# autonomousvision/unimatch

Measured on NVIDIA B200. Metric: image-pairs/sec @480x832 gmflow-scale2-refine6; EPE vs reference, higher is better.
Workload: dtype fp32

## Files before the change

include/unimatch_sm100.h:

```cpp
#ifndef UNIMATCH_SM100_H_
#define UNIMATCH_SM100_H_

#include <stdint.h>

#ifdef __cplusplus
extern "C" {
#endif

#define UM_OK 0
#define UM_EINVAL (-22)
#define UM_ECUDA (-5)

#define UM_FEATURE_DIM 128

int um_abi_version(void);
const char* um_build_info(void);
const char* um_last_error(void);
int64_t um_launch_count(void);

#define UM_MASK_NONE 0
#define UM_MASK_SWIN 1
#define UM_MASK_CAUSAL 2

typedef struct um_attn_geom {
// ... 7 lines not shown
                        int32_t n_streams, int32_t kv_shift,
                        int64_t ldq, int64_t ldk, int64_t ldv, int64_t ldo,
                        const um_attn_geom* geom, void* workspace, int64_t workspace_bytes, int32_t flags,
                        void* stream);
#define UM_ATTN_FORCE_CUDA_CORES 1
int64_t um_window_attention_workspace(const um_attn_geom* geom, int32_t n_streams);
void um_debug_set_dump(float* device_buffer);

int32_t um_attention_planes_lp(const um_attn_geom* geom);
int um_window_attention_planes(const void* q_planes, const void* k_planes, const void* v_planes, float* out, int64_t ldo,
                               void* out_split, int64_t split_plane_stride, int32_t n_streams, int32_t kv_shift,
                               const um_attn_geom* geom, void* stream);

#define UM_VALUE_TENSOR 0
#define UM_VALUE_COORDS 1
#define UM_VALUE_XCOORD 2
#define UM_POST_NONE 0
#define UM_POST_MINUS_OWN 1
#define UM_POST_OWN_MINUS 2

int um_softmax_expectation(const float* q, const float* k, const float* values, float* out,
                           int32_t n_streams, int32_t n_total, int32_t kv_shift,
                           int64_t ldq, int64_t ldk, int32_t vdim, int32_t value_mode, int32_t post_op,
                           const um_attn_geom* geom, void* workspace, int64_t workspace_bytes, int32_t flags,
                           void* stream);
int64_t um_softmax_expectation_workspace(const um_attn_geom* geom, int32_t n_total, int32_t value_mode);

int um_local_corr_softmax(const float* f0, const float* f1, float* flow,
                          int32_t batch, int32_t h, int32_t w, int32_t ry, int32_t rx, int32_t stereo,
                          void* stream);

int um_local_corr_volume(const float* f0, const float* f1, const float* flow, float* corr,
                         int32_t batch, int32_t h, int32_t w, int32_t radius, int32_t flow_dim, void* stream);

int um_flow_warp(const float* f, const float* flow, float* out,
                 int32_t batch, int32_t h, int32_t w, int32_t flow_dim, void* stream);

int um_fb_consistency(const float* fwd_flow, const float* bwd_flow, float alpha, float beta, float* fwd_occ,
                      float* bwd_occ, int32_t batch, int32_t h, int32_t w, void* stream);

int um_propagate_local(const float* q, const float* k, const float* flow, float* out,
                       int32_t batch, int32_t h, int32_t w, int32_t radius, int32_t flow_dim,
                       int64_t ldq, int64_t ldk, void* stream);

int um_depth_corr_softmax(const float* f0, const float* f1, const float* Kmat, const float* Kinv,
                          const float* pose, const float* cand, float* out,
                          int32_t batch, int32_t h, int32_t w, int32_t num_cand, int32_t from_argmax,
                          void* stream);

int um_add_position(const float* x, const float* table, float* out,
                    int32_t n_streams, int32_t h, int32_t w, int32_t wh, int32_t ww, void* stream);

int um_layernorm_residual(const float* x, const float* residual, const float* gamma, const float* beta,
                          float* out, int64_t rows, int64_t ldx, int64_t ldr, int64_t ldo, void* stream);

int um_convex_upsample(const float* flow, const float* mask, float* up,
                       int32_t batch, int32_t h, int32_t w, int32_t flow_dim, int32_t factor, float mult,
                       void* stream);

int um_upsample2x(const float* flow, float* out, int32_t batch, int32_t h, int32_t w, int32_t flow_dim,
                  float mult, void* stream);

int um_resize_bilinear(const float* in, float* out, int32_t batch, int32_t channels, int32_t h_in, int32_t w_in,
                       int32_t h_out, int32_t w_out, const float* scale, int32_t flip_x, void* stream);

int um_gru_rh(const float* r_pre, int64_t ldr, const float* h, int64_t ldh, float* rh, int64_t ldo, int64_t rows,
// ... 83 lines not shown
```

unimatch_b200/csrc/build.py:

```python
import hashlib
import os
import shutil
import subprocess
import sys

HERE = os.path.dirname(os.path.abspath(__file__))
ROOT = os.path.dirname(os.path.dirname(HERE))
LIB = os.path.join(os.path.dirname(HERE), "libunimatch_sm100.so")
SOURCES = ["um_api.cu", "um_attention_simt.cu", "um_attention_tc.cu", "um_attention_tc2.cu", "um_conv_tc.cu", "um_ffn_tc.cu", "um_local.cu", "um_local_stencil.cu", "um_misc.cu", "um_norm.cu", "um_stem.cu"]
FLAGS = ["-gencode", "arch=compute_100a,code=sm_100a", "-O3", "-lineinfo", "-std=c++17",
         "-Xcompiler", "-fPIC", "-Xcompiler", "-O2", "-I", os.path.join(ROOT, "include"), "-I", HERE]


def _nvcc():
    for c in (shutil.which("nvcc"), "/usr/local/cuda/bin/nvcc"):
        if c and os.path.exists(c):
            return c
    raise RuntimeError("nvcc not found: libunimatch_sm100.so cannot be built")


def have_nvcc():
    try:
        _nvcc()
        return True
    except RuntimeError:
        return False


if os.environ.get("UM_ATTN_DEBUG_BUILD") == "1":
    FLAGS = FLAGS + ["-DUM_ATTN_DEBUG=1"]


def _stamp():
    h = hashlib.sha256()
    h.update(" ".join(FLAGS).replace(ROOT, "").encode())
    for f in sorted(os.listdir(HERE)) + [os.path.join(ROOT, "include", "unimatch_sm100.h")]:
        p = f if os.path.isabs(f) else os.path.join(HERE, f)
        if p.endswith((".cu", ".cuh", ".h", "build.py")):
            h.update(open(p, "rb").read())
    return h.hexdigest()


# ... 55 lines not shown
```

unimatch_b200/csrc/um_local.cu:

```cuda
#include <limits.h>
#include <math_constants.h>

#include "um_common.cuh"

namespace {

constexpr float SQRT_C = 11.313708498984761f;
constexpr int PIX_PER_CTA = 32;

struct Tap { int x0, y0; float wnw, wne, wsw, wse; };

__device__ __forceinline__ float unnormalize(float g, int size) { return ((g + 1.0f) / 2.0f) * (float)(size - 1); }

__device__ __forceinline__ float norm_sample(float p, int size) { return 2.0f * p / (float)(size - 1) - 1.0f; }
__device__ __forceinline__ float norm_window(float p, int size) { float c = (float)(size - 1) / 2.0f; return (p - c) / c; }

__device__ __forceinline__ Tap make_tap(float ix, float iy) {
  Tap t;
  float fx = floorf(ix), fy = floorf(iy);
  t.x0 = (int)fx; t.y0 = (int)fy;
  float xe = fx + 1.0f, ye = fy + 1.0f;
  t.wnw = (xe - ix) * (ye - iy);
  t.wne = (ix - fx) * (ye - iy);
  t.wsw = (xe - ix) * (iy - fy);
  t.wse = (ix - fx) * (iy - fy);
  return t;
}

struct Vec16 { float4 v[4]; };

__device__ __forceinline__ Vec16 load_row(const float* row, int sub) {
  Vec16 r;
  const float4* p = reinterpret_cast<const float4*>(row);
#pragma unroll
  for (int i = 0; i < 4; ++i) r.v[i] = __ldg(p + sub + 8 * i);
  return r;
}
__device__ __forceinline__ void store_row(float* row, int sub, const Vec16& r) {
  float4* p = reinterpret_cast<float4*>(row);
#pragma unroll
  for (int i = 0; i < 4; ++i) p[sub + 8 * i] = r.v[i];
}
__device__ __forceinline__ Vec16 zero16() {
  Vec16 r;
#pragma unroll
  for (int i = 0; i < 4; ++i) r.v[i] = make_float4(0.f, 0.f, 0.f, 0.f);
  return r;
}
__device__ __forceinline__ void axpy(Vec16& acc, float w, const Vec16& x) {
#pragma unroll
  for (int i = 0; i < 4; ++i) {
    acc.v[i].x = fmaf(w, x.v[i].x, acc.v[i].x); acc.v[i].y = fmaf(w, x.v[i].y, acc.v[i].y);
    acc.v[i].z = fmaf(w, x.v[i].z, acc.v[i].z); acc.v[i].w = fmaf(w, x.v[i].w, acc.v[i].w);
  }
}
__device__ __forceinline__ float dot_partial(const Vec16& a, const Vec16& b) {
  float s = 0.f;
#pragma unroll
  for (int i = 0; i < 4; ++i) {
    s = fmaf(a.v[i].x, b.v[i].x, s); s = fmaf(a.v[i].y, b.v[i].y, s);
    s = fmaf(a.v[i].z, b.v[i].z, s); s = fmaf(a.v[i].w, b.v[i].w, s);
  }
  return s;
}
__device__ __forceinline__ float reduce8(float s) {
  const unsigned gmask = 0xFFu << (threadIdx.x & 24);
  s += __shfl_xor_sync(gmask, s, 4);
  s += __shfl_xor_sync(gmask, s, 2);
  s += __shfl_xor_sync(gmask, s, 1);
  return s;
}

__device__ __forceinline__ Vec16 sample(const float* img, int h, int w, const Tap& t, int sub) {
  Vec16 acc = zero16();
  const bool xl = (t.x0 >= 0 && t.x0 < w), xr = (t.x0 + 1 >= 0 && t.x0 + 1 < w);
  const bool yt = (t.y0 >= 0 && t.y0 < h), yb = (t.y0 + 1 >= 0 && t.y0 + 1 < h);
  if (yt && xl && t.wnw != 0.0f) axpy(acc, t.wnw, load_row(img + ((long long)t.y0 * w + t.x0) * UM_C, sub));
  if (yt && xr && t.wne != 0.0f) axpy(acc, t.wne, load_row(img + ((long long)t.y0 * w + t.x0 + 1) * UM_C, sub));
  if (yb && xl && t.wsw != 0.0f) axpy(acc, t.wsw, load_row(img + ((long long)(t.y0 + 1) * w + t.x0) * UM_C, sub));
  if (yb && xr && t.wse != 0.0f) axpy(acc, t.wse, load_row(img + ((long long)(t.y0 + 1) * w + t.x0 + 1) * UM_C, sub));
  return acc;
}

__device__ __forceinline__ void read_flow(const float* flow, long long pix, int flow_dim, float* u, float* v) {
  if (flow_dim == 2) { float2 f = __ldg(reinterpret_cast<const float2*>(flow) + pix); *u = f.x; *v = f.y; }
  else { *u = -__ldg(flow + pix); *v = 0.0f; }
}

__global__ void __launch_bounds__(256) flow_warp_kernel(const float* __restrict__ f, const float* __restrict__ flow,
                                                        float* __restrict__ out, int h, int w, int flow_dim,
                                                        long long npix) {
  const int sub = threadIdx.x & 7;
  const long long pix = (long long)blockIdx.x * PIX_PER_CTA + (threadIdx.x >> 3);
  if (pix >= npix) return;
  const long long hw = (long long)h * w;
  const int b = (int)(pix / hw);
  const int rem = (int)(pix - (long long)b * hw);
  const int y = rem / w, x = rem - y * w;
  float u, v;
  read_flow(flow, pix, flow_dim, &u, &v);
  const float px = (float)x + u, py = (float)y + v;
  Tap t = make_tap(unnormalize(norm_sample(px, w), w), unnormalize(norm_sample(py, h), h));
  Vec16 r = sample(f + (long long)b * hw * UM_C, h, w, t, sub);
  store_row(out + pix * UM_C, sub, r);
}

__global__ void __launch_bounds__(256) local_corr_softmax_kernel(const float* __restrict__ f0, const float* __restrict__ f1,
                                                                 float* __restrict__ out, int h, int w, int ry, int rx,
                                                                 int stereo, long long npix) {
  const int sub = threadIdx.x & 7;
  const long long pix = (long long)blockIdx.x * PIX_PER_CTA + (threadIdx.x >> 3);
  if (pix >= npix) return;
  const long long hw = (long long)h * w;
  const int b = (int)(pix / hw);
  const int rem = (int)(pix - (long long)b * hw);
  const int y = rem / w, x = rem - y * w;
  const Vec16 a = load_row(f0 + pix * UM_C, sub);
  const float* img = f1 + (long long)b * hw * UM_C;
  float m = -CUDART_INF_F, l = 0.f, ax = 0.f, ay = 0.f;
// ... 275 lines not shown
```

unimatch_b200/ops.py:

```python
import ctypes
import os

import torch

_HERE = os.path.dirname(os.path.abspath(__file__))
LIB_PATH = os.path.join(_HERE, "libunimatch_sm100.so")

SYMBOLS = [
    "um_abi_version", "um_build_info", "um_last_error", "um_launch_count",
    "um_window_attention", "um_window_attention_workspace", "um_attention_planes_lp", "um_window_attention_planes", "um_debug_set_dump", "um_softmax_expectation", "um_softmax_expectation_workspace",
    "um_local_corr_softmax", "um_local_corr_volume", "um_flow_warp", "um_fb_consistency", "um_propagate_local", "um_depth_corr_softmax",
    "um_conv2d_tc", "um_ffn_tc", "um_conv7x7_small", "um_split_planes", "um_instance_norm_scratch_floats", "um_instance_norm_stats", "um_instance_norm_apply", "um_add_position", "um_layernorm_residual", "um_convex_upsample", "um_upsample2x", "um_resize_bilinear", "um_gru_rh", "um_gru_update",
]

MASK_NONE, MASK_SWIN, MASK_CAUSAL = 0, 1, 2
VALUE_TENSOR, VALUE_COORDS, VALUE_XCOORD = 0, 1, 2
POST_NONE, POST_MINUS_OWN, POST_OWN_MINUS = 0, 1, 2


FORCE_CUDA_CORES = 1
_force_cuda_cores = False


def set_force_cuda_cores(flag):
    global _force_cuda_cores
    _force_cuda_cores = bool(flag)


ACT_NONE, ACT_RELU, ACT_TANH, ACT_SIGMOID, ACT_GELU = 0, 1, 2, 3, 4
CONV_LINEAR, CONV_GRU_ZR, CONV_GRU_Q, CONV_LN = 0, 1, 2, 3


class AttnGeom(ctypes.Structure):
    _fields_ = [(n, ctypes.c_int32) for n in ("h", "w", "kh", "kw", "sh", "sw", "mask_mode")]


class ConvDesc(ctypes.Structure):
    _fields_ = [("src", ctypes.c_void_p * 2), ("cin_p", ctypes.c_int32 * 2), ("nsrc", ctypes.c_int32),
                ("batch", ctypes.c_int32), ("h", ctypes.c_int32), ("w", ctypes.c_int32),
                ("weights", ctypes.c_void_p), ("bias", ctypes.c_void_p),
                ("kh", ctypes.c_int32), ("kw", ctypes.c_int32), ("pad_h", ctypes.c_int32), ("pad_w", ctypes.c_int32),
                ("cout", ctypes.c_int32), ("cout_p", ctypes.c_int32), ("bn", ctypes.c_int32),
                ("mode", ctypes.c_int32), ("act", ctypes.c_int32),
                ("out_f32", ctypes.c_void_p), ("ld_f32", ctypes.c_int64), ("off_f32", ctypes.c_int32),
# ... 5 lines not shown
                ("win_dst", ctypes.c_void_p), ("win_c0", ctypes.c_int32), ("win_c1", ctypes.c_int32),
                ("win_lp", ctypes.c_int32), ("win_streams", ctypes.c_int32), ("win_geom", AttnGeom),
                ("pre", ctypes.c_void_p), ("ld_pre", ctypes.c_int64)]


class FfnDesc(ctypes.Structure):
    _fields_ = [("src", ctypes.c_void_p * 2), ("src_plane_stride", ctypes.c_int64), ("rows", ctypes.c_int64),
                ("w1", ctypes.c_void_p), ("w2", ctypes.c_void_p), ("hidden", ctypes.c_int32),
                ("residual", ctypes.c_void_p), ("ld_res", ctypes.c_int64), ("gamma", ctypes.c_void_p), ("beta", ctypes.c_void_p),
                ("out_f32", ctypes.c_void_p), ("ld_f32", ctypes.c_int64), ("out_split", ctypes.c_void_p),
                ("split_plane_stride", ctypes.c_int64)]


def _load():
    from .csrc.build import build, have_nvcc
    if have_nvcc():
        build()
    elif not os.path.exists(LIB_PATH):
        raise ImportError("libunimatch_sm100.so is missing and nvcc is not available to build it")
    lib = ctypes.CDLL(LIB_PATH)
    missing = [s for s in SYMBOLS if not hasattr(lib, s)]
    if missing:
        raise ImportError("libunimatch_sm100.so lacks symbols %s (stale build? run python unimatch_b200/csrc/build.py --force)" % missing)
    lib.um_build_info.restype = ctypes.c_char_p
    lib.um_last_error.restype = ctypes.c_char_p
    lib.um_launch_count.restype = ctypes.c_int64
    P, I, L, F = ctypes.c_void_p, ctypes.c_int32, ctypes.c_int64, ctypes.c_float
    G = ctypes.POINTER(AttnGeom)
    sig = {
        "um_window_attention": [P, P, P, P, I, I, L, L, L, L, G, P, L, I, P],
        "um_softmax_expectation": [P, P, P, P, I, I, I, L, L, I, I, I, G, P, L, I, P],
        "um_local_corr_softmax": [P, P, P, I, I, I, I, I, I, P],
        "um_local_corr_volume": [P, P, P, P, I, I, I, I, I, P],
        "um_flow_warp": [P, P, P, I, I, I, I, P],
        "um_fb_consistency": [P, P, F, F, P, P, I, I, I, P],
        "um_propagate_local": [P, P, P, P, I, I, I, I, I, L, L, P],
        "um_depth_corr_softmax": [P, P, P, P, P, P, P, I, I, I, I, I, P],
        "um_add_position": [P, P, P, I, I, I, I, I, P],
        "um_layernorm_residual": [P, P, P, P, P, L, L, L, L, P],
        "um_convex_upsample": [P, P, P, I, I, I, I, I, F, P],
        "um_upsample2x": [P, P, I, I, I, I, F, P],
        "um_gru_rh": [P, L, P, L, P, L, L, P],
        "um_gru_update": [P, L, P, L, P, L, P, L, L, P],
    }
    lib.um_window_attention_workspace.argtypes = [G, I]
    lib.um_window_attention_workspace.restype = ctypes.c_int64
    lib.um_softmax_expectation_workspace.argtypes = [G, I, I]
    lib.um_softmax_expectation_workspace.restype = ctypes.c_int64
    lib.um_conv2d_tc.argtypes = [ctypes.POINTER(ConvDesc), P]
    lib.um_conv2d_tc.restype = ctypes.c_int
    lib.um_ffn_tc.argtypes = [ctypes.POINTER(FfnDesc), P]
    lib.um_ffn_tc.restype = ctypes.c_int
    lib.um_split_planes.argtypes = [P, L, I, L, P, I, I, L, P]
    lib.um_attention_planes_lp.argtypes = [G]
    lib.um_attention_planes_lp.restype = ctypes.c_int32
    lib.um_window_attention_planes.argtypes = [P, P, P, P, L, P, L, I, I, G, P]
    lib.um_window_attention_planes.restype = ctypes.c_int
    lib.um_split_planes.restype = ctypes.c_int
    FP = ctypes.POINTER(ctypes.c_float)
    lib.um_conv7x7_small.argtypes = [P, P, I, I, I, I, I, I, I, P, P, I, I, FP, FP, P, L, P, I, P]
    lib.um_conv7x7_small.restype = ctypes.c_int
    lib.um_instance_norm_scratch_floats.argtypes = [I, I]
    lib.um_instance_norm_scratch_floats.restype = ctypes.c_int64
    lib.um_instance_norm_stats.argtypes = [P, L, I, I, I, P, P, P]
    lib.um_instance_norm_stats.restype = ctypes.c_int
    lib.um_instance_norm_apply.argtypes = [P, L, P, I, P, L, P, I, P, L, P, I, I, I, I, I, P]
# ... 134 lines not shown
    return out


softmax_expectation = _define(
    "softmax_expectation(Tensor q, Tensor k, Tensor? values, int n_streams, int kv_shift, int vdim, int value_mode, "
    "int post_op, int h, int w, int kh, int kw, int mask_mode) -> Tensor", _softmax_expectation)


def _local_corr_softmax(f0, f1, h, w, ry, rx, stereo):
    _f32c(f0, "f0"), _f32c(f1, "f1")
    b = f0.shape[0]
    out = torch.empty((b, h, w, 1 if stereo else 2), device=f0.device, dtype=torch.float32)
    _check(LIB.um_local_corr_softmax(_p(f0), _p(f1), _p(out), b, h, w, ry, rx, int(stereo), _stream()),
           "um_local_corr_softmax")
    return out


local_corr_softmax = _define("local_corr_softmax(Tensor f0, Tensor f1, int h, int w, int ry, int rx, bool stereo) -> Tensor",
                             _local_corr_softmax)


def _local_corr_volume(f0, f1, flow, h, w, radius):
    _f32c(f0, "f0"), _f32c(f1, "f1"), _f32c(flow, "flow")
    b = f0.shape[0]
    k = (2 * radius + 1) ** 2
    out = torch.empty((b, h, w, k), device=f0.device, dtype=torch.float32)
    _check(LIB.um_local_corr_volume(_p(f0), _p(f1), _p(flow), _p(out), b, h, w, radius, flow.shape[-1], _stream()),
           "um_local_corr_volume")
    return out


local_corr_volume = _define("local_corr_volume(Tensor f0, Tensor f1, Tensor flow, int h, int w, int radius) -> Tensor",
                            _local_corr_volume)


def _flow_warp(f, flow, h, w):
    _f32c(f, "f"), _f32c(flow, "flow")
    out = torch.empty_like(f)
    _check(LIB.um_flow_warp(_p(f), _p(flow), _p(out), f.shape[0], h, w, flow.shape[-1], _stream()), "um_flow_warp")
    return out


flow_warp = _define("flow_warp(Tensor f, Tensor flow, int h, int w) -> Tensor", _flow_warp)


def _fb_consistency(fwd_flow, bwd_flow, alpha, beta):
    _f32c(fwd_flow, "fwd_flow"), _f32c(bwd_flow, "bwd_flow")
    if fwd_flow.dim() != 4 or fwd_flow.shape[1] != 2 or fwd_flow.shape != bwd_flow.shape:
        raise ValueError("fb_consistency: flows must be planar [B,2,H,W] of equal shape")
    b, _, h, w = fwd_flow.shape
    fwd_occ = torch.empty((b, h, w), device=fwd_flow.device, dtype=torch.float32)
    bwd_occ = torch.empty_like(fwd_occ)
    _check(LIB.um_fb_consistency(_p(fwd_flow), _p(bwd_flow), float(alpha), float(beta), _p(fwd_occ), _p(bwd_occ), b, h, w,
                                 _stream()), "um_fb_consistency")
    return fwd_occ, bwd_occ


fb_consistency = _define("fb_consistency(Tensor fwd_flow, Tensor bwd_flow, float alpha, float beta) -> (Tensor, Tensor)",
                         _fb_consistency)


def _propagate_local(q, k, flow, h, w, radius):
    ldq, ldk = _rows(q, "q"), _rows(k, "k")
    _f32c(flow, "flow")
    b = q.shape[0]
    out = torch.empty_like(flow)
# ... 299 lines not shown
```

unimatch_b200/unimatch.py:

```python
import math
from contextlib import contextmanager

import torch
import torch.nn as nn

from . import ops
from .spec import param_spec

_OPS = torch.ops.unimatch_sm100


import os as _os
_FUSED_FFN = _os.environ.get("UM_FUSED_FFN", "1") != "0"


def _bn256(b, h, w):
    return 128 if (b * ((h + 7) // 8) * ((w + 15) // 16)) % 2 == 0 else 256



class _Node(nn.Module):
    """Parameter container; gives the flat spec table the reference's dotted state_dict names."""


def _attach(root, key, param):
    parts = key.split(".")
    node = root
    for name in parts[:-1]:
        if name not in node._modules:
            node.add_module(name, _Node())
        node = node._modules[name]
    node.register_parameter(parts[-1], param)


def _sine_table(wh, ww):
    y = torch.arange(1, wh + 1, dtype=torch.float32)
    x = torch.arange(1, ww + 1, dtype=torch.float32)
    y = y / (float(wh) + 1e-6) * (2 * math.pi)
    x = x / (float(ww) + 1e-6) * (2 * math.pi)
    n = torch.arange(64, dtype=torch.float32)
    dim_t = 10000 ** (2 * torch.div(n, 2, rounding_mode="floor") / 64)
    even = (torch.arange(64) % 2 == 0)

    def enc(v):
        a = v[:, None] / dim_t
        return torch.where(even, a.sin(), a.cos())
# ... 398 lines not shown
                                        ops.VALUE_TENSOR, ops.POST_NONE, h, wd, 1, 1, ops.MASK_NONE).view(nb, h, wd, fd)

    class _RefineState:
        pass

    def _stage_refine_setup(self, P, feat0, b, h, w):
        T = P["tc"]
        dev = feat0.device
        st = self._RefineState()
        z16 = lambda cp: torch.empty((2, b, h, w, cp), device=dev, dtype=torch.float16)
        st.corr_s = self._zero_padded("corr", (2, b, h, w, 128), dev)
        st.cor1_s, st.cf_s, st.flo1_s = z16(256), z16(256), z16(128)
        st.inp_s, st.mfx_s = z16(128), z16(128)
        st.h0_s, st.h1_s, st.h2_s, st.rh_s, st.fh_s = z16(128), z16(128), z16(128), z16(128), z16(256)
        f0_s = z16(128)
        _OPS.split_planes(feat0, f0_s, 0)
        f32 = lambda cc: torch.empty((b, h, w, cc), device=dev)
        st.net0, st.z, st.h1, st.h2 = f32(128), f32(128), f32(128), f32(128)
        C, LIN, NONE = self._conv, ops.CONV_LINEAR, ops.ACT_NONE
        C(f0_s, None, *T["proj_net"], 1, 1, 0, 0, 128, 128, LIN, ops.ACT_TANH, st.net0, 0, st.h0_s, 0, None, None)
        C(f0_s, None, *T["proj_inp"], 1, 1, 0, 0, 128, 128, LIN, ops.ACT_RELU, None, 0, st.inp_s, 0, None, None)
        st.pre_zr1, st.pre_q1, st.pre_zr2, st.pre_q2 = f32(256), f32(128), f32(256), f32(128)
        bn_zr = _bn256(b, h, w)
        C(st.h0_s, st.inp_s, *T["zr1_fix"], 1, 5, 0, 2, 256, bn_zr, LIN, NONE, st.pre_zr1, 0, None, 0, None, None)
        C(st.inp_s, None, *T["q1_fix"], 1, 5, 0, 2, 128, 128, LIN, NONE, st.pre_q1, 0, None, 0, None, None)
        C(st.inp_s, None, *T["zr2_fix"], 5, 1, 2, 0, 256, bn_zr, LIN, NONE, st.pre_zr2, 0, None, 0, None, None)
        C(st.inp_s, None, *T["q2_fix"], 5, 1, 2, 0, 128, 128, LIN, NONE, st.pre_q2, 0, None, 0, None, None)
        return st

    def _update_block(self, P, st, corr, flow, want_mask):
        T, w = P["tc"], P["raw"]
        fd = T["fd"]
        C, L, R = self._conv, ops.CONV_LINEAR, ops.ACT_RELU
        b, h, wd, _ = corr.shape
        dev = corr.device
        bn_zr = bn_fh = _bn256(b, h, wd)
        _OPS.split_planes(corr, st.corr_s, 0)
        C(st.corr_s, None, *T["convc1"], 1, 1, 0, 0, 256, 256, L, R, None, 0, st.cor1_s, 0, None, None)
        C(st.cor1_s, None, *T["convc2"], 3, 3, 1, 1, 192, 96 if bn_zr == 128 else 192, L, R, None, 0, st.cf_s, 0, None, None)
        _OPS.conv7x7_small(flow, None, False, w["refine.encoder.convf1.weight"], w["refine.encoder.convf1.bias"], 1, True,
                           None, None, None, st.flo1_s)
        C(st.flo1_s, None, *T["convf2"], 3, 3, 1, 1, 64, 64, L, R, None, 0, st.cf_s, 192, None, None)
        C(st.cf_s, None, *T["conv"], 3, 3, 1, 1, 128 - fd, 128, L, R, None, 0, st.mfx_s, 0, None, None)
        _OPS.split_planes(flow, st.mfx_s, 128 - fd)
        Z, Q = ops.CONV_GRU_ZR, ops.CONV_GRU_Q
        kw = dict(gamma=None, beta=None, stride=1, rows=0, win_dst=None, win_geom=None, win_c0=0, win_c1=0, win_streams=0)
        C(st.mfx_s, None, T["zr1_var"], None, 1, 5, 0, 2, 256, bn_zr, Z, 0, st.z, 0, st.rh_s, 0, st.net0, None, pre=st.pre_zr1, **kw)
        C(st.rh_s, st.mfx_s, T["q1_var"], None, 1, 5, 0, 2, 128, 128, Q, 0, st.h1, 0, st.h1_s, 0, st.net0, st.z, pre=st.pre_q1, **kw)
        C(st.h1_s, st.mfx_s, T["zr2_var"], None, 5, 1, 2, 0, 256, bn_zr, Z, 0, st.z, 0, st.rh_s, 0, st.h1, None, pre=st.pre_zr2, **kw)
        C(st.rh_s, st.mfx_s, T["q2_var"], None, 5, 1, 2, 0, 128, 128, Q, 0, st.h2, 0, st.h2_s, 0, st.h1, st.z, pre=st.pre_q2, **kw)
        C(st.h2_s, None, *T["fh1"], 3, 3, 1, 1, 256, bn_fh, L, R, None, 0, st.fh_s, 0, None, None)
        delta = torch.empty((b, h, wd, fd), device=dev)
        C(st.fh_s, None, *T["fh2"], 3, 3, 1, 1, fd, 16, L, ops.ACT_NONE, delta, 0, None, 0, None, None)
        mask = None
        if want_mask and "mask0" in T:
            C(st.h2_s, None, *T["mask0"], 3, 3, 1, 1, 256, bn_fh, L, R, None, 0, st.fh_s, 0, None, None)
            nm = w["refine.mask.2.weight"].shape[0]
            mask = torch.empty((b, h, wd, nm), device=dev)
            C(st.fh_s, None, *T["mask2"], 1, 1, 0, 0, nm, 64, L, ops.ACT_NONE, mask, 0, None, 0, None, None)
        return st.h2, mask, delta

    def _stage_refine_iter(self, P, rst, g0, g1, flow, task, want_mask, depth=None):
        h, wd = flow.shape[1], flow.shape[2]
        if task == "depth":
            Kr, pr, min_depth, max_depth = depth
            cflow = self._rigid_flow(flow, Kr.float(), pr.float(), h, wd)
        else:
            cflow = flow.contiguous()
        with self._section("refine_corr_volume"):
            corr = _OPS.local_corr_volume(g0, g1, cflow, h, wd, 4)
        with self._section("refine_update_block"):
            _, mask, delta = self._update_block(P, rst, corr, flow.contiguous(), want_mask)
        if task == "depth":
            flow = (flow - delta).clamp(min=min_depth, max=max_depth)
        else:
            flow = flow + delta
        if task == "stereo":
            flow = flow.clamp(min=0)
        return flow, mask

    def _stage_upsample_learned(self, P, flow2, feat, factor, mult):
        U = P["up"]
        b, h, w, _ = feat.shape
        dev = feat.device
        C = self._conv
        src = self._zero_padded("upsampler", (2, b, h, w, 192), dev)
        _OPS.split_planes(feat.contiguous(), src, 0)
        _OPS.split_planes(flow2.contiguous(), src, 128)
        mid = torch.empty((2, b, h, w, 256), device=dev, dtype=torch.float16)
        C(src, None, *U["c0"], 3, 3, 1, 1, 256, _bn256(b, h, w), ops.CONV_LINEAR, ops.ACT_RELU, None, 0, mid, 0, None, None)
        m = torch.empty((b, h, w, U["nm"]), device=dev)
        C(mid, None, *U["c2"], 1, 1, 0, 0, U["nm"], U["bn2"], ops.CONV_LINEAR, ops.ACT_NONE, m, 0, None, 0, None, None)
        return _OPS.convex_upsample(flow2.contiguous(), m, factor, float(mult))

    @staticmethod
    def _rigid_flow(inv_depth, K, pose, h, w):
        b = inv_depth.shape[0]
        dev = inv_depth.device
        ys, xs = torch.meshgrid(torch.arange(h, device=dev, dtype=torch.float32),
                                torch.arange(w, device=dev, dtype=torch.float32), indexing="ij")
        grid = torch.stack([xs, ys, torch.ones_like(xs)], dim=0).view(1, 3, -1).expand(b, 3, h * w)
        depth = (1.0 / inv_depth.view(b, 1, h * w))
        pts = torch.inverse(K).bmm(grid) * depth
# ... 114 lines not shown
```

Measured before the change: 157.1.

## Compute refine local correlation volume on tensor cores from fp16 split planes

```diff
diff --git a/include/unimatch_sm100.h b/include/unimatch_sm100.h
--- a/include/unimatch_sm100.h
+++ b/include/unimatch_sm100.h
@@ -63,6 +63,9 @@
 
 int um_local_corr_volume(const float* f0, const float* f1, const float* flow, float* corr,
                          int32_t batch, int32_t h, int32_t w, int32_t radius, int32_t flow_dim, void* stream);
+int um_local_corr_volume_planes(const void* f0_planes, const void* f1_planes, const float* flow, float* corr,
+                                void* out_split, int32_t cp_split, int32_t off_split, int32_t batch, int32_t h, int32_t w,
+                                int32_t radius, int32_t flow_dim, int32_t* fallback_tiles, void* stream);
 
 int um_flow_warp(const float* f, const float* flow, float* out,
                  int32_t batch, int32_t h, int32_t w, int32_t flow_dim, void* stream);
diff --git a/unimatch_b200/csrc/build.py b/unimatch_b200/csrc/build.py
--- a/unimatch_b200/csrc/build.py
+++ b/unimatch_b200/csrc/build.py
@@ -7,7 +7,7 @@
 HERE = os.path.dirname(os.path.abspath(__file__))
 ROOT = os.path.dirname(os.path.dirname(HERE))
 LIB = os.path.join(os.path.dirname(HERE), "libunimatch_sm100.so")
-SOURCES = ["um_api.cu", "um_attention_simt.cu", "um_attention_tc.cu", "um_attention_tc2.cu", "um_conv_tc.cu", "um_ffn_tc.cu", "um_local.cu", "um_local_stencil.cu", "um_misc.cu", "um_norm.cu", "um_stem.cu"]
+SOURCES = ["um_api.cu", "um_attention_simt.cu", "um_attention_tc.cu", "um_attention_tc2.cu", "um_conv_tc.cu", "um_ffn_tc.cu", "um_local.cu", "um_local_tc.cu", "um_local_stencil.cu", "um_misc.cu", "um_norm.cu", "um_stem.cu"]
 FLAGS = ["-gencode", "arch=compute_100a,code=sm_100a", "-O3", "-lineinfo", "-std=c++17",
          "-Xcompiler", "-fPIC", "-Xcompiler", "-O2", "-I", os.path.join(ROOT, "include"), "-I", HERE]
 
diff --git a/unimatch_b200/csrc/um_local.cu b/unimatch_b200/csrc/um_local.cu
--- a/unimatch_b200/csrc/um_local.cu
+++ b/unimatch_b200/csrc/um_local.cu
@@ -2,40 +2,14 @@
 #include <math_constants.h>
 
 #include "um_common.cuh"
+#include "um_local_tap.cuh"
 
 namespace {
 
-constexpr float SQRT_C = 11.313708498984761f;
+using namespace um::local;
+
 constexpr int PIX_PER_CTA = 32;
 
-struct Tap { int x0, y0; float wnw, wne, wsw, wse; };
-
-__device__ __forceinline__ float unnormalize(float g, int size) { return ((g + 1.0f) / 2.0f) * (float)(size - 1); }
-
-__device__ __forceinline__ float norm_sample(float p, int size) { return 2.0f * p / (float)(size - 1) - 1.0f; }
-__device__ __forceinline__ float norm_window(float p, int size) { float c = (float)(size - 1) / 2.0f; return (p - c) / c; }
-
-__device__ __forceinline__ Tap make_tap(float ix, float iy) {
-  Tap t;
-  float fx = floorf(ix), fy = floorf(iy);
-  t.x0 = (int)fx; t.y0 = (int)fy;
-  float xe = fx + 1.0f, ye = fy + 1.0f;
-  t.wnw = (xe - ix) * (ye - iy);
-  t.wne = (ix - fx) * (ye - iy);
-  t.wsw = (xe - ix) * (iy - fy);
-  t.wse = (ix - fx) * (iy - fy);
-  return t;
-}
-
-struct Vec16 { float4 v[4]; };
-
-__device__ __forceinline__ Vec16 load_row(const float* row, int sub) {
-  Vec16 r;
-  const float4* p = reinterpret_cast<const float4*>(row);
-#pragma unroll
-  for (int i = 0; i < 4; ++i) r.v[i] = __ldg(p + sub + 8 * i);
-  return r;
-}
 __device__ __forceinline__ void store_row(float* row, int sub, const Vec16& r) {
   float4* p = reinterpret_cast<float4*>(row);
 #pragma unroll
@@ -54,23 +28,6 @@
     acc.v[i].z = fmaf(w, x.v[i].z, acc.v[i].z); acc.v[i].w = fmaf(w, x.v[i].w, acc.v[i].w);
   }
 }
-__device__ __forceinline__ float dot_partial(const Vec16& a, const Vec16& b) {
-  float s = 0.f;
-#pragma unroll
-  for (int i = 0; i < 4; ++i) {
-    s = fmaf(a.v[i].x, b.v[i].x, s); s = fmaf(a.v[i].y, b.v[i].y, s);
-    s = fmaf(a.v[i].z, b.v[i].z, s); s = fmaf(a.v[i].w, b.v[i].w, s);
-  }
-  return s;
-}
-__device__ __forceinline__ float reduce8(float s) {
-  const unsigned gmask = 0xFFu << (threadIdx.x & 24);
-  s += __shfl_xor_sync(gmask, s, 4);
-  s += __shfl_xor_sync(gmask, s, 2);
-  s += __shfl_xor_sync(gmask, s, 1);
-  return s;
-}
-
 __device__ __forceinline__ Vec16 sample(const float* img, int h, int w, const Tap& t, int sub) {
   Vec16 acc = zero16();
   const bool xl = (t.x0 >= 0 && t.x0 < w), xr = (t.x0 + 1 >= 0 && t.x0 + 1 < w);
@@ -80,11 +37,6 @@
   if (yb && xl && t.wsw != 0.0f) axpy(acc, t.wsw, load_row(img + ((long long)(t.y0 + 1) * w + t.x0) * UM_C, sub));
   if (yb && xr && t.wse != 0.0f) axpy(acc, t.wse, load_row(img + ((long long)(t.y0 + 1) * w + t.x0 + 1) * UM_C, sub));
   return acc;
-}
-
-__device__ __forceinline__ void read_flow(const float* flow, long long pix, int flow_dim, float* u, float* v) {
-  if (flow_dim == 2) { float2 f = __ldg(reinterpret_cast<const float2*>(flow) + pix); *u = f.x; *v = f.y; }
-  else { *u = -__ldg(flow + pix); *v = 0.0f; }
 }
 
 __global__ void __launch_bounds__(256) flow_warp_kernel(const float* __restrict__ f, const float* __restrict__ flow,
diff --git a/unimatch_b200/csrc/um_local_tap.cuh b/unimatch_b200/csrc/um_local_tap.cuh
--- /dev/null
+++ b/unimatch_b200/csrc/um_local_tap.cuh
@@ -0,0 +1,76 @@
+#pragma once
+#include "um_common.cuh"
+
+namespace um {
+namespace local {
+
+constexpr float SQRT_C = 11.313708498984761f;
+
+struct Tap { int x0, y0; float wnw, wne, wsw, wse; };
+
+__device__ __forceinline__ float unnormalize(float g, int size) { return ((g + 1.0f) / 2.0f) * (float)(size - 1); }
+
+__device__ __forceinline__ float norm_sample(float p, int size) { return 2.0f * p / (float)(size - 1) - 1.0f; }
+__device__ __forceinline__ float norm_window(float p, int size) { float c = (float)(size - 1) / 2.0f; return (p - c) / c; }
+
+__device__ __forceinline__ Tap make_tap(float ix, float iy) {
+  Tap t;
+  float fx = floorf(ix), fy = floorf(iy);
+  t.x0 = (int)fx; t.y0 = (int)fy;
+  float xe = fx + 1.0f, ye = fy + 1.0f;
+  t.wnw = (xe - ix) * (ye - iy);
+  t.wne = (ix - fx) * (ye - iy);
+  t.wsw = (xe - ix) * (iy - fy);
+  t.wse = (ix - fx) * (iy - fy);
+  return t;
+}
+
+__device__ __forceinline__ void read_flow(const float* flow, long long pix, int flow_dim, float* u, float* v) {
+  if (flow_dim == 2) { float2 f = __ldg(reinterpret_cast<const float2*>(flow) + pix); *u = f.x; *v = f.y; }
+  else { *u = -__ldg(flow + pix); *v = 0.0f; }
+}
+
+__device__ __forceinline__ Tap corr_center_tap(const float* flow, long long pix, int flow_dim, int x, int y, int h, int w) {
+  float u, v;
+  read_flow(flow, pix, flow_dim, &u, &v);
+  const float cx = unnormalize(norm_window((float)x + u, w), w);
+  const float cy = unnormalize(norm_window((float)y + v, h), h);
+  return make_tap(cx, cy);
+}
+
+__device__ __forceinline__ float blend(float nw, float ne, float sw, float se, const Tap& t) {
+  float r = nw * t.wnw;
+  r = fmaf(ne, t.wne, r);
+  r = fmaf(sw, t.wsw, r);
+  r = fmaf(se, t.wse, r);
+  return r / SQRT_C;
+}
+
+struct Vec16 { float4 v[4]; };
+
+__device__ __forceinline__ Vec16 load_row(const float* row, int sub) {
+  Vec16 r;
+  const float4* p = reinterpret_cast<const float4*>(row);
+#pragma unroll
+  for (int i = 0; i < 4; ++i) r.v[i] = __ldg(p + sub + 8 * i);
+  return r;
+}
+__device__ __forceinline__ float dot_partial(const Vec16& a, const Vec16& b) {
+  float s = 0.f;
+#pragma unroll
+  for (int i = 0; i < 4; ++i) {
+    s = fmaf(a.v[i].x, b.v[i].x, s); s = fmaf(a.v[i].y, b.v[i].y, s);
+    s = fmaf(a.v[i].z, b.v[i].z, s); s = fmaf(a.v[i].w, b.v[i].w, s);
+  }
+  return s;
+}
+__device__ __forceinline__ float reduce8(float s) {
+  const unsigned gmask = 0xFFu << (threadIdx.x & 24);
+  s += __shfl_xor_sync(gmask, s, 4);
+  s += __shfl_xor_sync(gmask, s, 2);
+  s += __shfl_xor_sync(gmask, s, 1);
+  return s;
+}
+
+}
+}
diff --git a/unimatch_b200/csrc/um_local_tc.cu b/unimatch_b200/csrc/um_local_tc.cu
--- /dev/null
+++ b/unimatch_b200/csrc/um_local_tc.cu
@@ -0,0 +1,387 @@
+#include <limits.h>
+
+#include "um_common.cuh"
+#include "um_local_tap.cuh"
+#include "um_tc.cuh"
+
+namespace um {
+
+using namespace tc;
+using namespace local;
+
+namespace {
+
+constexpr int TW = 16, TH = 8;
+constexpr int R = 4, GRID = 2 * R + 2, NOUT = (2 * R + 1) * (2 * R + 1);
+constexpr int CW = 32, CH = 8;
+constexpr int CSTEP = CW - GRID + 1;
+constexpr int MAX_CHUNKS = 6;
+constexpr int MAX_SPREAD = 256;
+constexpr int STAGES = 2;
+constexpr int NEPI = 8;
+constexpr int NTHREADS = 64 + 32 * NEPI;
+constexpr int INFO_SLOTS = 4;
+constexpr int ROWBUF_LD = 33;
+constexpr uint32_t A_BYTES = 4 * 16384;
+constexpr uint32_t STAGE_BYTES = 32768;
+constexpr uint32_t STAGING_BYTES = 128 * NOUT * 4;
+constexpr uint32_t ROWBUF_BYTES = NEPI * 32 * ROWBUF_LD * 4;
+constexpr uint32_t TAIL_BYTES = 256;
+constexpr uint32_t SMEM_BYTES = A_BYTES + STAGES * STAGE_BYTES + STAGING_BYTES + ROWBUF_BYTES + TAIL_BYTES;
+static_assert(SMEM_BYTES <= 232448, "shared memory budget");
+
+struct TileInfo { int X0, Y0, nr, nc; };
+
+struct CorrParams {
+  int B, H, W, tiles_x, tiles_y, ntiles, flow_dim;
+  const float* flow;
+  const __half* f0; const __half* f1; long long plane;
+  float* out_f32;
+  __half* out_split; int cp_split, off_split; long long plane_split;
+  int* fallback;
+};
+
+__device__ __forceinline__ bool tile_pixel_tap(const CorrParams& p, int b, int y0, int x0, int m, Tap* t) {
+  const int y = y0 + (m >> 4), x = x0 + (m & 15);
+  if (y >= p.H || x >= p.W) return false;
+  *t = corr_center_tap(p.flow, ((long long)b * p.H + y) * p.W + x, p.flow_dim, x, y, p.H, p.W);
+  return true;
+}
+
+__device__ __forceinline__ Vec16 load_row_planes(const __half* hi, long long plane, int sub) {
+  Vec16 r;
+  const uint2* ph = reinterpret_cast<const uint2*>(hi);
+  const uint2* pl = reinterpret_cast<const uint2*>(hi + plane);
+#pragma unroll
+  for (int i = 0; i < 4; ++i) {
+    const uint2 h = __ldg(ph + sub + 8 * i), l = __ldg(pl + sub + 8 * i);
+    const float2 h01 = __half22float2(*reinterpret_cast<const __half2*>(&h.x));
+    const float2 h23 = __half22float2(*reinterpret_cast<const __half2*>(&h.y));
+    const float2 l01 = __half22float2(*reinterpret_cast<const __half2*>(&l.x));
+    const float2 l23 = __half22float2(*reinterpret_cast<const __half2*>(&l.y));
+    r.v[i] = make_float4(h01.x + l01.x, h01.y + l01.y, h23.x + l23.x, h23.y + l23.y);
+  }
+  return r;
+}
+
+__global__ void __launch_bounds__(NTHREADS, 1)
+local_corr_tc_kernel(const __grid_constant__ CUtensorMap map_a, const __grid_constant__ CUtensorMap map_b, CorrParams p) {
+  extern __shared__ __align__(1024) uint8_t smem[];
+  uint8_t* sa = smem;
+  uint8_t* sb = smem + A_BYTES;
+  float* staging = reinterpret_cast<float*>(smem + A_BYTES + STAGES * STAGE_BYTES);
+  float* rowbufs = reinterpret_cast<float*>(smem + A_BYTES + STAGES * STAGE_BYTES + STAGING_BYTES);
+  uint64_t* bars = reinterpret_cast<uint64_t*>(smem + A_BYTES + STAGES * STAGE_BYTES + STAGING_BYTES + ROWBUF_BYTES);
+  uint64_t* full = bars;
+  uint64_t* empty = full + STAGES;
+  uint64_t* acc_full = empty + STAGES;
+  uint64_t* acc_empty = acc_full + 2;
+  uint64_t* a_full = acc_empty + 2;
+  uint64_t* a_empty = a_full + 1;
+  uint64_t* info_full = a_empty + 1;
+  uint64_t* info_empty = info_full + INFO_SLOTS;
+  uint32_t* tmem_slot = reinterpret_cast<uint32_t*>(info_empty + INFO_SLOTS);
+  TileInfo* info = reinterpret_cast<TileInfo*>(bars + 24);
+  static_assert((2 * STAGES + 6 + 2 * INFO_SLOTS) * 8 + 4 <= 24 * 8 && 24 * 8 + INFO_SLOTS * 16 <= TAIL_BYTES, "tail layout");
+
+  const int warp = threadIdx.x >> 5, lane = threadIdx.x & 31;
+  if (threadIdx.x == 0) {
+    for (int i = 0; i < STAGES; ++i) { mbar_init(full + i, 1); mbar_init(empty + i, 1); }
+    for (int i = 0; i < 2; ++i) { mbar_init(acc_full + i, 1); mbar_init(acc_empty + i, 32 * NEPI); }
+    mbar_init(a_full, 1); mbar_init(a_empty, 1);
+    for (int i = 0; i < INFO_SLOTS; ++i) { mbar_init(info_full + i, 1); mbar_init(info_empty + i, 1 + 32 * NEPI); }
+    fence_barrier_init();
+  }
+  if (warp == 0 && lane == 0) { tma_prefetch_desc(&map_a); tma_prefetch_desc(&map_b); }
+  if (warp == 1) tmem_alloc(tmem_slot, 512);
+  tc_fence_before();
+  __syncthreads();
+  tc_fence_after();
+  const uint32_t tmem = *tmem_slot;
+  const int tiles_img = p.tiles_x * p.tiles_y;
+
+  if (warp == 0) {
+    int it = 0, na = 0, lt = 0;
+    for (int t = blockIdx.x; t < p.ntiles; t += gridDim.x, ++lt) {
+      const int b = t / tiles_img, rem = t - b * tiles_img;
+      const int y0 = (rem / p.tiles_x) * TH, x0 = (rem % p.tiles_x) * TW;
+      int mnx = INT_MAX, mxx = INT_MIN, mny = INT_MAX, mxy = INT_MIN;
+#pragma unroll
+      for (int i = 0; i < 4; ++i) {
+        Tap tp;
+        if (tile_pixel_tap(p, b, y0, x0, lane + 32 * i, &tp)) {
+          mnx = min(mnx, tp.x0); mxx = max(mxx, tp.x0); mny = min(mny, tp.y0); mxy = max(mxy, tp.y0);
+        }
+      }
+      mnx = __reduce_min_sync(0xffffffffu, mnx); mxx = __reduce_max_sync(0xffffffffu, mxx);
+      mny = __reduce_min_sync(0xffffffffu, mny); mxy = __reduce_max_sync(0xffffffffu, mxy);
+      const long long sx = (long long)mxx - mnx, sy = (long long)mxy - mny;
+      TileInfo ti{mnx - R, mny - R, 0, 0};
+      const bool boxed = sx <= MAX_SPREAD && sy <= MAX_SPREAD && mnx > -(1 << 24) && mnx < (1 << 24) &&
+                         mny > -(1 << 24) && mny < (1 << 24);
+      if (boxed) {
+        const int nc = (int)sx / CSTEP + 1, nr = ((int)sy + GRID + CH - 1) / CH;
+        if (nc * nr <= MAX_CHUNKS) { ti.nr = nr; ti.nc = nc; }
+      }
+      const int slot = lt % INFO_SLOTS;
+      mbar_wait(info_empty + slot, ((lt / INFO_SLOTS) & 1) ^ 1);
+      if (lane == 0) {
+        info[slot] = ti;
+        mbar_arrive(info_full + slot);
+        if (ti.nr == 0 && p.fallback) atomicAdd(p.fallback, 1);
+      }
+      __syncwarp();
+      if (ti.nr == 0) continue;
+      mbar_wait(a_empty, (na & 1) ^ 1);
+      ++na;
+      if (elect_one()) {
+        mbar_arrive_expect_tx(a_full, A_BYTES);
+#pragma unroll
+        for (int kc = 0; kc < 2; ++kc)
+#pragma unroll
+          for (int part = 0; part < 2; ++part)
+            tma_load_4d(sa + (kc * 2 + part) * 16384, &map_a, a_full, kc * 64, x0, y0, part * p.B + b);
+      }
+      __syncwarp();
+      for (int cr = 0; cr < ti.nr; ++cr)
+        for (int cc = 0; cc < ti.nc; ++cc)
+          for (int s = 0; s < 4; ++s, ++it) {
+            const int st = it % STAGES;
+            mbar_wait(empty + st, ((it / STAGES) & 1) ^ 1);
+            if (elect_one()) {
+              mbar_arrive_expect_tx(full + st, STAGE_BYTES);
+              tma_load_4d(sb + st * STAGE_BYTES, &map_b, full + st, (s >> 1) * 64, ti.X0 + cc * CSTEP, ti.Y0 + cr * CH,
+                          (s & 1) * p.B + b);
+            }
+            __syncwarp();
+          }
+    }
+  } else if (warp == 1) {
+    constexpr uint32_t IDESC = idesc_f16(128, 256, 0, 0);
+    int it = 0, ch = 0, na = 0, lt = 0;
+    for (int t = blockIdx.x; t < p.ntiles; t += gridDim.x, ++lt) {
+      const int slot = lt % INFO_SLOTS;
+      mbar_wait(info_full + slot, (lt / INFO_SLOTS) & 1);
+      const TileInfo ti = info[slot];
+      __syncwarp();
+      if (elect_one()) mbar_arrive(info_empty + slot);
+      __syncwarp();
+      if (ti.nr == 0) continue;
+      mbar_wait(a_full, na & 1);
+      ++na;
+      tc_fence_after();
+      const int nch = ti.nr * ti.nc;
+      for (int c = 0; c < nch; ++c, ++ch) {
+        const int buf = ch & 1;
+        mbar_wait(acc_empty + buf, ((ch >> 1) & 1) ^ 1);
+        tc_fence_after();
+        const uint32_t d = tmem + buf * 256;
+        for (int s = 0; s < 4; ++s, ++it) {
+          const int st = it % STAGES, kc = s >> 1;
+          mbar_wait(full + st, (it / STAGES) & 1);
+          tc_fence_after();
+          const uint32_t b_base = smem_u32(sb + st * STAGE_BYTES);
+          const uint32_t a_hi = smem_u32(sa + (kc * 2) * 16384), a_lo = a_hi + 16384;
+          if (elect_one()) {
+            if ((s & 1) == 0) {
+#pragma unroll
+              for (int ks = 0; ks < 4; ++ks) umma_f16(d, desc_kmajor(a_lo + ks * 32), desc_kmajor(b_base + ks * 32), IDESC, s > 0 || ks > 0);
+#pragma unroll
+              for (int ks = 0; ks < 4; ++ks) umma_f16(d, desc_kmajor(a_hi + ks * 32), desc_kmajor(b_base + ks * 32), IDESC, true);
+            } else {
+#pragma unroll
+              for (int ks = 0; ks < 4; ++ks) umma_f16(d, desc_kmajor(a_hi + ks * 32), desc_kmajor(b_base + ks * 32), IDESC, true);
+            }
+            umma_commit(empty + st);
+            if (s == 3 && c == nch - 1) umma_commit(a_empty);
+            if (s == 3) umma_commit(acc_full + buf);
+          }
+          __syncwarp();
+        }
+      }
+    }
+  } else {
+    const int quarter = warp & 3, ew = warp - 2, half = ew >> 2;
+    const int iy_lo = half ? GRID / 2 : 0, iy_hi = half ? GRID - 1 : GRID / 2;
+    const int m = quarter * 32 + lane;
+    const int e = ew * 32 + lane;
+    float* rowbuf = rowbufs + ew * 32 * ROWBUF_LD;
+    auto epi_sync = [&]() { asm volatile("bar.sync 1, %0;" ::"n"(32 * NEPI) : "memory"); };
+    int ch = 0, lt = 0;
+    for (int t = blockIdx.x; t < p.ntiles; t += gridDim.x, ++lt) {
+      const int b = t / tiles_img, rem = t - b * tiles_img;
+      const int y0 = (rem / p.tiles_x) * TH, x0 = (rem % p.tiles_x) * TW;
+      const int slot = lt % INFO_SLOTS;
+      mbar_wait(info_full + slot, (lt / INFO_SLOTS) & 1);
+      const TileInfo ti = info[slot];
+      mbar_arrive(info_empty + slot);
+      if (ti.nr > 0) {
+        Tap tp{};
+        const bool valid = tile_pixel_tap(p, b, y0, x0, m, &tp);
+        const int oxr = tp.x0 - R - ti.X0, oyr = tp.y0 - R - ti.Y0;
+        const int mycc = valid ? oxr / CSTEP : -1;
+        const int off = oxr - mycc * CSTEP;
+        float* orow = staging + m * NOUT;
+        float prev[GRID], cur[GRID];
+        for (int cr = 0; cr < ti.nr; ++cr) {
+          for (int cc = 0; cc < ti.nc; ++cc, ++ch) {
+            const int buf = ch & 1;
+            mbar_wait(acc_full + buf, (ch >> 1) & 1);
+            tc_fence_after();
+            const uint32_t taddr = tmem + ((uint32_t)(quarter * 32) << 16) + buf * 256;
+#pragma unroll 1
+            for (int ry = 0; ry < CH; ++ry) {
+              const int iy = cr * CH + ry - oyr;
+              const bool need = cc == mycc && iy >= iy_lo && iy <= iy_hi;
+              if (!__any_sync(0xffffffffu, need)) continue;
+              float v[32];
+              tmem_ld32(taddr + ry * 32, v);
+              tmem_wait_ld();
+#pragma unroll
+              for (int i = 0; i < 32; ++i) rowbuf[lane * ROWBUF_LD + i] = v[i];
+              __syncwarp();
+              if (need) {
+#pragma unroll
+                for (int j = 0; j < GRID; ++j) cur[j] = rowbuf[lane * ROWBUF_LD + off + j];
+                if (iy > iy_lo) {
+                  float* o = orow + (iy - 1) * (GRID - 1);
+#pragma unroll
+                  for (int ix = 0; ix < GRID - 1; ++ix) o[ix] = blend(prev[ix], prev[ix + 1], cur[ix], cur[ix + 1], tp);
+                }
+#pragma unroll
+                for (int j = 0; j < GRID; ++j) prev[j] = cur[j];
+              }
+              __syncwarp();
+            }
+            tc_fence_before();
+            mbar_arrive(acc_empty + buf);
+          }
+        }
+      } else {
+        const int sub = lane & 7, grp = lane >> 3;
+        float* dots = rowbuf + grp * GRID * GRID;
+        const __half* img = p.f1 + (long long)b * p.H * p.W * UM_C;
+#pragma unroll 1
+        for (int pass = 0; pass < 128 / (4 * NEPI); ++pass) {
+          const int mm = pass * 4 * NEPI + ew * 4 + grp;
+          Tap tq;
+          const bool ok = tile_pixel_tap(p, b, y0, x0, mm, &tq);
+          if (ok) {
+            const long long pix = ((long long)b * p.H + y0 + (mm >> 4)) * p.W + x0 + (mm & 15);
+            const Vec16 a = load_row_planes(p.f0 + pix * UM_C, p.plane, sub);
+            for (int iy = 0; iy < GRID; ++iy) {
+              const int yy = tq.y0 - R + iy;
+              for (int ix = 0; ix < GRID; ++ix) {
+                const int xx = tq.x0 - R + ix;
+                float d = 0.f;
+                if (yy >= 0 && yy < p.H && xx >= 0 && xx < p.W)
+                  d = dot_partial(a, load_row_planes(img + ((long long)yy * p.W + xx) * UM_C, p.plane, sub));
+                d = reduce8(d);
+                if (sub == 0) dots[iy * GRID + ix] = d;
+              }
+            }
+          }
+          __syncwarp();
+          if (ok) {
+            for (int k = sub; k < NOUT; k += 8) {
+              const int iy = k / (GRID - 1), ix = k - iy * (GRID - 1);
+              const float* d = dots + iy * GRID + ix;
+              staging[mm * NOUT + k] = blend(d[0], d[1], d[GRID], d[GRID + 1], tq);
+            }
+          }
+          __syncwarp();
+        }
+      }
+      epi_sync();
+      const int nvx = min(TW, p.W - x0);
+      for (int py = 0; py < TH && y0 + py < p.H; ++py) {
+        const long long pix0 = ((long long)b * p.H + y0 + py) * p.W + x0;
+        const int n = nvx * NOUT;
+        const float* src = staging + py * TW * NOUT;
+        if (p.out_f32) {
+          float* dst = p.out_f32 + pix0 * NOUT;
+#pragma unroll 4
+          for (int i = e; i < n; i += 32 * NEPI) dst[i] = src[i];
+        }
+        if (p.out_split) {
+#pragma unroll 4
+          for (int i = e; i < n; i += 32 * NEPI) {
+            const int px = i / NOUT, k = i - px * NOUT;
+            __half hi, lo;
+            split_f16(src[i], &hi, &lo);
+            __half* dh = p.out_split + (pix0 + px) * p.cp_split + p.off_split + k;
+            dh[0] = hi;
+            dh[p.plane_split] = lo;
+          }
+        }
+      }
+      epi_sync();
+    }
+  }
+
+  tc_fence_before();
+  __syncthreads();
+  if (warp == 1) {
+    tc_fence_after();
+    tmem_dealloc(tmem, 512);
+  }
+}
+
+int make_map_chunk(CUtensorMap* map, const void* base, uint64_t W, uint64_t H, uint64_t NB) {
+  PFN_encodeTiled enc = get_encode_tiled();
+  if (!enc) { set_error("cuTensorMapEncodeTiled unavailable"); return UM_ECUDA; }
+  cuuint64_t dims[4] = {UM_C, W, H, NB};
+  cuuint64_t strides[3] = {UM_C * 2, UM_C * W * 2, UM_C * W * H * 2};
+  cuuint32_t box[4] = {64, CW, CH, 1};
+  cuuint32_t estr[4] = {1, 1, 1, 1};
+  CUresult r = enc(map, CU_TENSOR_MAP_DATA_TYPE_FLOAT16, 4, const_cast<void*>(base), dims, strides, box, estr,
+                   CU_TENSOR_MAP_INTERLEAVE_NONE, CU_TENSOR_MAP_SWIZZLE_128B, CU_TENSOR_MAP_L2_PROMOTION_L2_256B,
+                   CU_TENSOR_MAP_FLOAT_OOB_FILL_NONE);
+  if (r != CUDA_SUCCESS) { set_error("cuTensorMapEncodeTiled(corr chunk) failed (%d)", (int)r); return UM_ECUDA; }
+  return UM_OK;
+}
+
+}
+}
+
+extern "C" {
+
+int um_local_corr_volume_planes(const void* f0_planes, const void* f1_planes, const float* flow, float* corr,
+                                void* out_split, int32_t cp_split, int32_t off_split, int32_t batch, int32_t h, int32_t w,
+                                int32_t radius, int32_t flow_dim, int32_t* fallback_tiles, void* stream) {
+  using namespace um;
+  UM_REQUIRE(f0_planes && f1_planes && flow && batch > 0 && h > 1 && w > 1, "um_local_corr_volume_planes: bad arguments");
+  UM_REQUIRE(radius == R, "um_local_corr_volume_planes: only radius 4 is built (unimatch.py:308-313 uses local_radius=4)");
+  UM_REQUIRE(flow_dim == 1 || flow_dim == 2, "um_local_corr_volume_planes: flow_dim must be 1 or 2");
+  UM_REQUIRE(corr || out_split, "um_local_corr_volume_planes: no output");
+  UM_REQUIRE(((reinterpret_cast<uintptr_t>(f0_planes) | reinterpret_cast<uintptr_t>(f1_planes)) & 15) == 0,
+             "um_local_corr_volume_planes: feature planes must be 16-byte aligned");
+  if (out_split)
+    UM_REQUIRE(off_split >= 0 && cp_split >= off_split + NOUT, "um_local_corr_volume_planes: split output needs cp >= off + 81");
+  CorrParams p{};
+  p.B = batch; p.H = h; p.W = w; p.flow_dim = flow_dim;
+  p.tiles_x = (w + TW - 1) / TW; p.tiles_y = (h + TH - 1) / TH;
+  p.ntiles = p.tiles_x * p.tiles_y * batch;
+  p.flow = flow;
+  p.f0 = reinterpret_cast<const __half*>(f0_planes); p.f1 = reinterpret_cast<const __half*>(f1_planes);
+  p.plane = (long long)batch * h * w * UM_C;
+  p.out_f32 = corr;
+  p.out_split = reinterpret_cast<__half*>(out_split); p.cp_split = cp_split; p.off_split = off_split;
+  p.plane_split = (long long)batch * h * w * cp_split;
+  p.fallback = fallback_tiles;
+  CUtensorMap ma, mb;
+  int rc;
+  if ((rc = make_map_4d_f16(&ma, f0_planes, UM_C, w, h, 2ull * batch, 1))) return rc;
+  if ((rc = make_map_chunk(&mb, f1_planes, w, h, 2ull * batch))) return rc;
+  cudaStream_t st = (cudaStream_t)stream;
+  if (fallback_tiles && cudaMemsetAsync(fallback_tiles, 0, sizeof(int32_t), st) != cudaSuccess)
+    return check_launch("um_local_corr_volume_planes(counter)");
+  static PerDeviceBytes configured;
+  if ((rc = ensure_smem(configured, local_corr_tc_kernel, SMEM_BYTES, "local_corr_tc"))) return rc;
+  const int sms = device_sm_count();
+  const int grid = p.ntiles < sms ? p.ntiles : sms;
+  local_corr_tc_kernel<<<grid, NTHREADS, SMEM_BYTES, st>>>(ma, mb, p);
+  return check_launch("um_local_corr_volume_planes");
+}
+
+}
diff --git a/unimatch_b200/ops.py b/unimatch_b200/ops.py
--- a/unimatch_b200/ops.py
+++ b/unimatch_b200/ops.py
@@ -9,7 +9,7 @@
 SYMBOLS = [
     "um_abi_version", "um_build_info", "um_last_error", "um_launch_count",
     "um_window_attention", "um_window_attention_workspace", "um_attention_planes_lp", "um_window_attention_planes", "um_debug_set_dump", "um_softmax_expectation", "um_softmax_expectation_workspace",
-    "um_local_corr_softmax", "um_local_corr_volume", "um_flow_warp", "um_fb_consistency", "um_propagate_local", "um_depth_corr_softmax",
+    "um_local_corr_softmax", "um_local_corr_volume", "um_local_corr_volume_planes", "um_flow_warp", "um_fb_consistency", "um_propagate_local", "um_depth_corr_softmax",
     "um_conv2d_tc", "um_ffn_tc", "um_conv7x7_small", "um_split_planes", "um_instance_norm_scratch_floats", "um_instance_norm_stats", "um_instance_norm_apply", "um_add_position", "um_layernorm_residual", "um_convex_upsample", "um_upsample2x", "um_resize_bilinear", "um_gru_rh", "um_gru_update",
 ]
 
@@ -81,6 +81,7 @@
         "um_softmax_expectation": [P, P, P, P, I, I, I, L, L, I, I, I, G, P, L, I, P],
         "um_local_corr_softmax": [P, P, P, I, I, I, I, I, I, P],
         "um_local_corr_volume": [P, P, P, P, I, I, I, I, I, P],
+        "um_local_corr_volume_planes": [P, P, P, P, P, I, I, I, I, I, I, I, P, P],
         "um_flow_warp": [P, P, P, I, I, I, I, P],
         "um_fb_consistency": [P, P, F, F, P, P, I, I, I, P],
         "um_propagate_local": [P, P, P, P, I, I, I, I, I, L, L, P],
@@ -281,6 +282,36 @@
 
 local_corr_volume = _define("local_corr_volume(Tensor f0, Tensor f1, Tensor flow, int h, int w, int radius) -> Tensor",
                             _local_corr_volume)
+
+
+def _local_corr_volume_planes(f0_planes, f1_planes, flow, h, w, radius, out_f32, out_split, off_split, fallback_tiles):
+    b = f0_planes.shape[1]
+    for t, name in ((f0_planes, "f0_planes"), (f1_planes, "f1_planes")):
+        if t.dtype != torch.float16 or not t.is_contiguous() or tuple(t.shape) != (2, b, h, w, 128):
+            raise RuntimeError("local_corr_volume_planes: %s must be contiguous fp16 planes [2, B, h, w, 128]" % name)
+    _f32c(flow, "flow")
+    if tuple(flow.shape[:3]) != (b, h, w):
+        raise RuntimeError("local_corr_volume_planes: flow must be [B, h, w, 1 or 2]")
+    k = (2 * radius + 1) ** 2
+    if out_f32 is not None:
+        _f32c(out_f32, "out_f32")
+        if tuple(out_f32.shape) != (b, h, w, k):
+            raise RuntimeError("local_corr_volume_planes: out_f32 must be [B, h, w, %d]" % k)
+    cp = 0
+    if out_split is not None:
+        if out_split.dtype != torch.float16 or not out_split.is_contiguous() or tuple(out_split.shape[:4]) != (2, b, h, w):
+            raise RuntimeError("local_corr_volume_planes: out_split must be contiguous fp16 planes [2, B, h, w, cp]")
+        cp = out_split.shape[-1]
+    if fallback_tiles is not None and (fallback_tiles.dtype != torch.int32 or fallback_tiles.numel() < 1):
+        raise RuntimeError("local_corr_volume_planes: fallback_tiles must be an int32 tensor")
+    _check(LIB.um_local_corr_volume_planes(_p(f0_planes), _p(f1_planes), _p(flow), _p(out_f32), _p(out_split), cp, off_split,
+                                           b, h, w, radius, flow.shape[-1], _p(fallback_tiles), _stream()),
+           "um_local_corr_volume_planes")
+
+
+local_corr_volume_planes = _define(
+    "local_corr_volume_planes(Tensor f0_planes, Tensor f1_planes, Tensor flow, int h, int w, int radius, Tensor(a!)? out_f32, "
+    "Tensor(b!)? out_split, int off_split, Tensor(c!)? fallback_tiles) -> ()", _local_corr_volume_planes)
 
 
 def _flow_warp(f, flow, h, w):
diff --git a/unimatch_b200/unimatch.py b/unimatch_b200/unimatch.py
--- a/unimatch_b200/unimatch.py
+++ b/unimatch_b200/unimatch.py
@@ -12,6 +12,7 @@
 
 import os as _os
 _FUSED_FFN = _os.environ.get("UM_FUSED_FFN", "1") != "0"
+_CORR_TC = _os.environ.get("UM_CORR_TC", "1") != "0"
 
 
 def _bn256(b, h, w):
@@ -476,10 +477,11 @@
         T, w = P["tc"], P["raw"]
         fd = T["fd"]
         C, L, R = self._conv, ops.CONV_LINEAR, ops.ACT_RELU
-        b, h, wd, _ = corr.shape
-        dev = corr.device
+        b, h, wd, _ = flow.shape
+        dev = flow.device
         bn_zr = bn_fh = _bn256(b, h, wd)
-        _OPS.split_planes(corr, st.corr_s, 0)
+        if corr is not None:
+            _OPS.split_planes(corr, st.corr_s, 0)
         C(st.corr_s, None, *T["convc1"], 1, 1, 0, 0, 256, 256, L, R, None, 0, st.cor1_s, 0, None, None)
         C(st.cor1_s, None, *T["convc2"], 3, 3, 1, 1, 192, 96 if bn_zr == 128 else 192, L, R, None, 0, st.cf_s, 0, None, None)
         _OPS.conv7x7_small(flow, None, False, w["refine.encoder.convf1.weight"], w["refine.encoder.convf1.bias"], 1, True,
@@ -504,6 +506,18 @@
             C(st.fh_s, None, *T["mask2"], 1, 1, 0, 0, nm, 64, L, ops.ACT_NONE, mask, 0, None, 0, None, None)
         return st.h2, mask, delta
 
+    @staticmethod
+    def _refine_feature_planes(rst, g0, g1):
+        cached = getattr(rst, "g_planes", None)
+        if cached is None or cached[0] is not g0 or cached[1] is not g1:
+            planes = []
+            for g in (g0, g1):
+                gs = torch.empty((2,) + tuple(g.shape), device=g.device, dtype=torch.float16)
+                _OPS.split_planes(g, gs, 0)
+                planes.append(gs)
+            rst.g_planes = (g0, g1, planes[0], planes[1])
+        return rst.g_planes[2], rst.g_planes[3]
+
     def _stage_refine_iter(self, P, rst, g0, g1, flow, task, want_mask, depth=None):
         h, wd = flow.shape[1], flow.shape[2]
         if task == "depth":
@@ -512,7 +526,12 @@
         else:
             cflow = flow.contiguous()
         with self._section("refine_corr_volume"):
-            corr = _OPS.local_corr_volume(g0, g1, cflow, h, wd, 4)
+            if _CORR_TC and g0.is_cuda:
+                g0_s, g1_s = self._refine_feature_planes(rst, g0, g1)
+                _OPS.local_corr_volume_planes(g0_s, g1_s, cflow, h, wd, 4, None, rst.corr_s, 0, None)
+                corr = None
+            else:
+                corr = _OPS.local_corr_volume(g0, g1, cflow, h, wd, 4)
         with self._section("refine_update_block"):
             _, mask, delta = self._update_block(P, rst, corr, flow.contiguous(), want_mask)
         if task == "depth":
```

Measured after the change: 164.6 (median of 6 runs). +4.8%, better.
